# RC4ML/Legion

Measured on AMD Instinct MI355X. Metric: sampled_edges_per_sec, higher is better.
Workload: dtype int32+f32(copy)

## Files before the change

### legion_amd/csrc/kernels_sample.hip

```cpp
#include "legion_core.h"
#include "draw_rule.h"

#include <cstdlib>

namespace lg {

__global__ void draw_batch_kernel(const int32_t* idx, const int32_t* deg, int32_t* out, int32_t n)
{
    int32_t i = blockIdx.x * blockDim.x + threadIdx.x;
    if (i < n) out[i] = draw_from_x(minstd_pow((uint32_t)idx[i] + 1u), deg[i]);
}

void launch_draw_batch(hipStream_t s, const int32_t* idx, const int32_t* deg, int32_t* out, int32_t n)
{
    if (n <= 0) return;
    draw_batch_kernel<<<(n + 255) / 256, 256, 0, s>>>(idx, deg, out, n);
    hipCheckError();
}

__device__ __forceinline__ int32_t floyd_draw(uint32_t x, int32_t deg, int32_t f, int32_t k)
{
    return draw_from_x(x, deg - f + k + 1);
}

template <typename T>
__device__ __forceinline__ void floyd_resolve(T* p, int32_t n, int32_t jbase)
{
    for (int32_t k = 1; k < n; k++) {
        const int32_t t = p[k];
        bool taken = false;
        for (int32_t i = 0; i < k; i++) taken |= (p[i] == t);
        if (taken) p[k] = jbase + k;
    }
}

__global__ void draw_distinct_batch_kernel(const int32_t* base, const int32_t* deg, int32_t f, int32_t* out, int32_t n)
{
    const int32_t i = blockIdx.x * blockDim.x + threadIdx.x;
    if (i >= n) return;
    const int32_t D = deg[i] > 0 ? deg[i] : 0;
    int32_t* p = out + (int64_t)i * f;
    for (int32_t k = 0; k < f; k++)
        p[k] = k >= D ? -1 : (D <= f ? k : floyd_draw(minstd_pow((uint32_t)(base[i] + k) + 1u), D, f, k));
    if (D > f) floyd_resolve(p, f, D - f);
}

void launch_draw_distinct_batch(hipStream_t s, const int32_t* base, const int32_t* deg, int32_t f, int32_t* out, int32_t n)
{
    if (n <= 0) return;
    draw_distinct_batch_kernel<<<(n + 255) / 256, 256, 0, s>>>(base, deg, f, out, n);
    hipCheckError();
}

__global__ void draw_weighted_batch_kernel(const int32_t* idx, const int64_t* row_start, const int32_t* deg, const float* cdf, int32_t* out, int32_t n)
{
    const int32_t i = blockIdx.x * blockDim.x + threadIdx.x;
    if (i >= n) return;
    const int32_t D = deg[i];
    int32_t pick = -1;
    if (D > 0) {
        const float* c = cdf + row_start[i];
        const float T = c[D - 1];
        if (T > 0.0f) {
            const double t = weighted_target(minstd_pow((uint32_t)idx[i] + 1u), T);
            int32_t lo = 0, m = D;
            while (m > 0) weighted_step(c[lo + (m >> 1)], t, lo, m);
            pick = min(lo, D - 1);
        }
    }
    out[i] = pick;
}

void launch_draw_weighted_batch(hipStream_t s, const int32_t* idx, const int64_t* row_start, const int32_t* deg, const float* cdf, int32_t* out, int32_t n)
{
    if (n <= 0) return;
    draw_weighted_batch_kernel<<<(n + 255) / 256, 256, 0, s>>>(idx, row_start, deg, cdf, out, n);
    hipCheckError();
}

struct BracketLane {
    LG_G int32_t* sampled_ids; LG_G int32_t* labels; LG_G int32_t* node_counter; LG_G int32_t* edge_counter;
    LG_G int32_t* hop_scratch; LG_G int32_t* node_slot;
    LG_G int32_t* known_cnt; LG_G int32_t* claim_cnt; int32_t lds_buckets;
    LG_G int32_t* counter_mirror;
};
__device__ __forceinline__ BracketLane bracket_lane(const LanePtrs& P)
{
    BracketLane L;
    L.sampled_ids = LG_GPTR(int32_t, P.sampled_ids); L.labels = LG_GPTR(int32_t, P.labels);
    L.node_counter = LG_GPTR(int32_t, P.node_counter); L.edge_counter = LG_GPTR(int32_t, P.edge_counter);
    L.hop_scratch = LG_GPTR(int32_t, P.hop_scratch); L.node_slot = LG_GPTR(int32_t, P.node_slot);
    L.known_cnt = LG_GPTR(int32_t, P.known_cnt); L.claim_cnt = LG_GPTR(int32_t, P.claim_cnt); L.lds_buckets = P.lds_buckets;
    L.counter_mirror = LG_GPTR(int32_t, P.counter_mirror);
    return L;
}

__device__ __forceinline__ void raise_error(LG_G int32_t* hop_scratch, LG_G int32_t* err_flag, int32_t bits)
{
    __hip_atomic_fetch_or(hop_scratch + HS_ERROR, bits, __ATOMIC_RELAXED, __HIP_MEMORY_SCOPE_AGENT);
    if (err_flag) __hip_atomic_fetch_or(err_flag, bits, __ATOMIC_RELAXED, __HIP_MEMORY_SCOPE_SYSTEM);
}

__global__ void batch_generate_kernel(SeedParams p, const LanePtrs* __restrict__ lanes)
{
    const BracketLane L = bracket_lane(lanes[blockIdx.y]);
    const int32_t idx = blockIdx.x * blockDim.x + threadIdx.x;
    const int32_t counter = (p.iter_state != nullptr ? p.iter_state[0] : p.counter0) + (int32_t)blockIdx.y;
    const int32_t size = ((int64_t)p.batch_size * (counter + 1) >= p.total_cap)
                             ? (p.total_cap - p.batch_size * counter) : p.batch_size;
    if (L.known_cnt != nullptr && idx < L.lds_buckets) L.known_cnt[idx] = 0;
    if (L.claim_cnt != nullptr && idx < L.lds_buckets) L.claim_cnt[idx * LG_CLAIM_CNT_STRIDE] = 0;
    if (idx < 16) {
        int32_t v = 0;
        if (idx == 1) v = size;
        if (idx == INTRABATCH_CON * 3) v = size;
        if (idx == INTRABATCH_CON * 3 - 1) v = p.hop_num;
        L.node_counter[idx] = v;
        L.edge_counter[idx] = 0;
        if (idx == 0) {
            L.hop_scratch[HS_RANGE] = 0;
            L.hop_scratch[HS_RANGE + 1] = size;
        }
    }
    if (idx < size) {
        const int64_t at = (int64_t)size * counter + idx;
        if (at >= p.total_cap) {
            L.sampled_ids[idx] = -1;
            L.labels[idx] = -1;
        } else {
            const int32_t src_id = p.all_ids[at % p.total_cap];
            L.sampled_ids[idx] = src_id;
            if (L.node_slot != nullptr) L.node_slot[idx] = LG_FS_UNKNOWN;
            L.labels[idx] = p.all_labels[at % p.total_cap];
        }
    }
}

void launch_batch_generate(hipStream_t s, const SeedParams& p, const LanePtrs* d_lanes, int32_t n_lanes)
{
    const int32_t n = p.batch_size > 256 ? p.batch_size : 256;
    batch_generate_kernel<<<dim3((n + 255) / 256, n_lanes), 256, 0, s>>>(p, d_lanes);
    hipCheckError();
}

typedef int32_t lg_v4i __attribute__((ext_vector_type(4)));
typedef int32_t lg_v2i __attribute__((ext_vector_type(2)));
template <int NB> __device__ __forceinline__ int64_t lg_claim_at(int32_t b, int32_t k)
{
    return ((((int64_t)(k >> LG_CLAIM_CHUNK_BITS) * NB) + b) << LG_CLAIM_CHUNK_BITS) + (k & (LG_CLAIM_CHUNK - 1));
}
struct SampleArgs {
    int32_t op_id, count, partition_count, max_slots;
    int32_t* const* csr_dst_node_ids;
    int32_t* const* csr_dst_x;
    const LG_G int32_t* col_full; const LG_G lg_v2i* colx_full;
    const LG_G RowHdr* row_hdr;
    bool last_hop, is_presc;
    LG_G unsigned long long* edge_access_time;
    LG_G unsigned long long* topo_transactions;
    LG_G int32_t* sampled_ids; LG_G int32_t* agg_src_ids; LG_G int32_t* agg_dst_ids; LG_G int32_t* agg_src_off; LG_G int32_t* agg_dst_off;
    LG_G char* tmp_part_ind; LG_G int32_t* node_counter; LG_G int32_t* edge_counter;
    LG_G int32_t* slot_dst; LG_G int32_t* slot_pos; LG_G int32_t* slot_fs; LG_G int32_t* node_slot; LG_G unsigned long long* tile_state; LG_G int32_t* hop_scratch;
    LG_G RowHdr* fh_edge;
    LG_G int32_t* err_flag;
    LG_G unsigned long long* claim_pairs; LG_G int32_t* run_off; LG_G int32_t* claim_cnt; int32_t claim_cap, ids_cap;
    LG_G unsigned long long* known_pairs; LG_G int32_t* known_cnt; int32_t known_cap;
    const LG_G int64_t* indptr_full; LG_G int32_t* slot_pick; LG_G int64_t* agg_edge_ids;
    const LG_G float* edge_cdf;
};


__device__ __forceinline__ RowHdr load_hdr(const LG_G RowHdr* p)
{
    const lg_v4i t = *(const LG_G lg_v4i*)p;
    RowHdr h;
    h.start = (int64_t)(((uint64_t)(uint32_t)t.y << 32) | (uint32_t)t.x);
    h.deg = t.z;
    h.slot = t.w;
    return h;
}
__device__ __forceinline__ void store_hdr(LG_G RowHdr* p, const RowHdr& h)
{
    lg_v4i t;
    t.x = (int32_t)(uint32_t)h.start;
    t.y = (int32_t)((uint64_t)h.start >> 32);
    t.z = h.deg;
    t.w = h.slot;
    *(LG_G lg_v4i*)p = t;
}

__device__ __forceinline__ SampleArgs lane_args(const HopParams& p, const LanePtrs* __restrict__ lanes)
{
    const LanePtrs& L = lanes[blockIdx.y];
    SampleArgs a;
    a.op_id = p.op_id; a.count = p.count; a.partition_count = p.partition_count; a.max_slots = p.max_slots;
    a.csr_dst_node_ids = p.csr_dst_node_ids; a.csr_dst_x = p.csr_dst_x;
    a.col_full = LG_GPTR(const int32_t, p.col_full); a.colx_full = LG_GPTR(const lg_v2i, p.colx_full); a.row_hdr = LG_GPTR(const RowHdr, p.row_hdr); a.last_hop = p.last_hop; a.is_presc = p.is_presc;
    a.edge_access_time = LG_GPTR(unsigned long long, p.edge_access_time);
    a.topo_transactions = LG_GPTR(unsigned long long, p.topo_transactions);
    a.sampled_ids = LG_GPTR(int32_t, L.sampled_ids); a.agg_src_ids = LG_GPTR(int32_t, L.agg_src_ids);
    a.agg_dst_ids = LG_GPTR(int32_t, L.agg_dst_ids); a.agg_src_off = LG_GPTR(int32_t, L.agg_src_off);
    a.agg_dst_off = LG_GPTR(int32_t, L.agg_dst_off); a.tmp_part_ind = LG_GPTR(char, L.tmp_part_ind);
    a.node_counter = LG_GPTR(int32_t, L.node_counter);
    a.edge_counter = LG_GPTR(int32_t, L.edge_counter); a.slot_dst = LG_GPTR(int32_t, L.slot_dst);
    a.slot_pos = LG_GPTR(int32_t, L.slot_pos);
    a.slot_fs = LG_GPTR(int32_t, L.slot_fs); a.node_slot = LG_GPTR(int32_t, L.node_slot); a.tile_state = LG_GPTR(unsigned long long, L.tile_state); a.hop_scratch = LG_GPTR(int32_t, L.hop_scratch);
    a.fh_edge = LG_GPTR(RowHdr, L.fh_edge);
    a.err_flag = LG_GPTR(int32_t, L.err_flag);
    a.claim_pairs = LG_GPTR(unsigned long long, L.claim_pairs);
    a.run_off = LG_GPTR(int32_t, L.run_off);
    a.claim_cnt = LG_GPTR(int32_t, L.claim_cnt); a.claim_cap = L.claim_cap; a.ids_cap = L.ids_cap;
    a.known_pairs = LG_GPTR(unsigned long long, L.known_pairs); a.known_cnt = LG_GPTR(int32_t, L.known_cnt); a.known_cap = L.known_cap;
    a.indptr_full = LG_GPTR(const int64_t, p.indptr_full); a.slot_pick = LG_GPTR(int32_t, L.slot_pick);
    a.agg_edge_ids = LG_GPTR(int64_t, L.agg_edge_ids);
    a.edge_cdf = LG_GPTR(const float, p.edge_cdf);
    return a;
}

struct HopGeom {
    const LG_G int32_t* frontier;
    int32_t frontier_len;
    int32_t frontier_off;
    int32_t total;
    int32_t ntiles;
    int32_t nsuper;
};

__device__ __forceinline__ HopGeom hop_geometry(const SampleArgs& a)
{
    HopGeom g;
    if (a.op_id == INTRABATCH_CON) {
        g.frontier = a.sampled_ids;
        g.frontier_len = a.node_counter[1];
        g.frontier_off = 0;
    } else {
        g.frontier_off = a.edge_counter[0];
        g.frontier = a.agg_src_ids + g.frontier_off;
        g.frontier_len = a.edge_counter[1];
    }
    int64_t total = (int64_t)(g.frontier_len > 0 ? g.frontier_len : 0) * a.count;
    if (total > a.max_slots) total = a.max_slots;
    g.total = (int32_t)total;
    g.ntiles = (g.total + LG_TILE - 1) / LG_TILE;
    g.nsuper = (g.total + LG_SUPER - 1) / LG_SUPER;
    return g;
}

#ifndef LG_SAMPLE_SGPRS
#define LG_SAMPLE_SGPRS 80
#endif
template <int BB, bool SINGLE, bool STAGED, SampleDraw DRAW, bool EIDS>
__global__ __launch_bounds__(LG_TILE) __attribute__((amdgpu_num_sgpr(LG_SAMPLE_SGPRS))) void sample_kernel(HopParams hp, const LanePtrs* __restrict__ lanes)
{
    constexpr int NB = 1 << BB;
    constexpr bool DISTINCT = DRAW == SampleDraw::Distinct, WEIGHTED = DRAW == SampleDraw::Weighted;
    const int32_t K = SINGLE ? 1 : hp.lds_k;
    static_assert(NB <= LG_TILE, "one thread per bucket in the prefix");
    const SampleArgs a = lane_args(hp, lanes);
    __shared__ RowHdr s_hdr[LG_SUPER];
    __shared__ int32_t s_pick[DISTINCT ? LG_SUPER + LG_DISTINCT_MAX_FANOUT - 1 : 1];
    __shared__ int32_t s_bcnt[NB], s_boff[SINGLE ? NB : 1], s_list[STAGED ? NB : 1];
    static_assert(!STAGED || (SINGLE && NB <= 64), "the staged form scans its buckets with one wave");
    static_assert(!WEIGHTED || LG_SLOTS_PER_LANE == 4, "the lock-step search below names its four slots");

    const HopGeom g = hop_geometry(a);
    const int32_t tid = threadIdx.x;
    const int32_t count = a.count;
    const bool seeds = (a.op_id == INTRABATCH_CON);
    const LG_G RowHdr* fh = a.fh_edge + g.frontier_off;

    const int32_t nparts = (g.nsuper + K - 1) / K;
    for (int32_t m = blockIdx.x; m < nparts; m += gridDim.x) {
        if (!SINGLE && tid < NB) s_bcnt[tid] = 0;
        for (int32_t sub = 0; sub < K; sub++) {
            const int32_t st = m * K + sub;
            if (st >= g.nsuper) break;
            const int32_t idx0 = st * LG_SUPER;
            const int32_t last = min(idx0 + LG_SUPER - 1, g.total - 1);
            const int32_t j0 = idx0 / count;
            const int32_t nsrc = last / count - j0 + 1;

            uint32_t x[LG_SLOTS_PER_LANE];
#pragma unroll
            for (int u = 0; u < LG_SLOTS_PER_LANE; u++) x[u] = minstd_pow((uint32_t)(idx0 + u * LG_TILE + tid) + 1u);

            unsigned long long tx = 0;
            for (int32_t t = tid; t < nsrc; t += LG_TILE) {
                RowHdr h;
                bool real = true;
                if (seeds) {
                    const int32_t src = g.frontier[j0 + t];
                    if (src >= 0) {
                        h = load_hdr(a.row_hdr + src);
                    } else {
                        h.start = 0; h.deg = 0; h.slot = a.partition_count;
                        real = false;
                    }
                } else {
                    h = load_hdr(fh + j0 + t);
                }
                s_hdr[t] = h;
                if (a.topo_transactions && real && (int64_t)(j0 + t) * count >= idx0)
                    tx += 1ull + (unsigned long long)min(count, (h.deg * 4 + 63) / 64);
                if (!a.is_presc)
                    a.tmp_part_ind[j0 + t] = (char)(h.slot == a.partition_count ? CACHEMISS_FLAG : h.slot);
            }
            if (a.topo_transactions) {
                for (int off = 32; off > 0; off >>= 1) tx += __shfl_down(tx, off);
                if ((tid & 63) == 0 && tx != 0)
                    __hip_atomic_fetch_add(a.topo_transactions, tx, __ATOMIC_RELAXED, __HIP_MEMORY_SCOPE_AGENT);
            }
            __syncthreads();

            if constexpr (DISTINCT) {
                const int32_t sbase = j0 * count;
#pragma unroll
                for (int u = 0; u < LG_SLOTS_PER_LANE; u++) {
                    const int32_t idx = idx0 + u * LG_TILE + tid;
                    if (idx < g.total) {
                        const int32_t q = idx / count;
                        const int32_t k = idx - q * count;
                        const int32_t deg = s_hdr[q - j0].deg;
                        if (deg > count) s_pick[idx - sbase] = floyd_draw(x[u], deg, count, k);
                    }
                }
                __syncthreads();
                for (int32_t t = tid; t < nsrc; t += LG_TILE) {
                    const int32_t deg = s_hdr[t].deg;
                    if (deg <= count) continue;
                    if (t == 0)
                        for (int32_t k = 0; k < idx0 - sbase; k++) s_pick[k] = floyd_draw(minstd_pow((uint32_t)(sbase + k) + 1u), deg, count, k);
                    floyd_resolve(s_pick + t * count, min(count, last + 1 - (j0 + t) * count), deg - count);
                }
                __syncthreads();
            }

            if (SINGLE && tid < NB) s_bcnt[tid] = 0;
            int32_t dst[LG_SLOTS_PER_LANE], fs[LG_SLOTS_PER_LANE];
            int32_t pk[EIDS ? LG_SLOTS_PER_LANE : 1];
            int32_t wpick[WEIGHTED ? LG_SLOTS_PER_LANE : 1];
            if constexpr (WEIGHTED) {
                const LG_G float* wc[LG_SLOTS_PER_LANE];
                int32_t wn[LG_SLOTS_PER_LANE], wlo[LG_SLOTS_PER_LANE], wdeg[LG_SLOTS_PER_LANE];
                double wt[LG_SLOTS_PER_LANE];
#pragma unroll
                for (int u = 0; u < LG_SLOTS_PER_LANE; u++) {
                    const int32_t idx = idx0 + u * LG_TILE + tid;
                    wn[u] = 0; wlo[u] = 0; wdeg[u] = 0; wc[u] = a.edge_cdf;
                    if (idx < g.total) {
                        const int32_t q = idx / count;
                        const RowHdr h = s_hdr[q - j0];
                        if (idx - q * count < h.deg) {
                            const int64_t base = h.slot == a.partition_count ? h.start : a.indptr_full[g.frontier[q]];
                            wc[u] = a.edge_cdf + base;
                            wdeg[u] = h.deg;
                        }
                    }
                }
                float wtot[LG_SLOTS_PER_LANE];
#pragma unroll
                for (int u = 0; u < LG_SLOTS_PER_LANE; u++) wtot[u] = wdeg[u] > 0 ? wc[u][wdeg[u] - 1] : 0.0f;
#pragma unroll
                for (int u = 0; u < LG_SLOTS_PER_LANE; u++) {
                    wt[u] = weighted_target(x[u], wtot[u]);
                    if (wtot[u] > 0.0f) wn[u] = wdeg[u];
                }
                while ((wn[0] | wn[1] | wn[2] | wn[3]) != 0) {
                    float v[LG_SLOTS_PER_LANE];
#pragma unroll
                    for (int u = 0; u < LG_SLOTS_PER_LANE; u++) v[u] = wn[u] > 0 ? wc[u][wlo[u] + (wn[u] >> 1)] : 0.0f;
#pragma unroll
                    for (int u = 0; u < LG_SLOTS_PER_LANE; u++)
                        if (wn[u] > 0) weighted_step(v[u], wt[u], wlo[u], wn[u]);
                }
#pragma unroll
                for (int u = 0; u < LG_SLOTS_PER_LANE; u++) wpick[u] = wtot[u] > 0.0f ? min(wlo[u], wdeg[u] - 1) : -1;
            }
#pragma unroll
            for (int u = 0; u < LG_SLOTS_PER_LANE; u++) {
                const int32_t idx = idx0 + u * LG_TILE + tid;
                dst[u] = -1;
                fs[u] = LG_FS_UNKNOWN;
                if constexpr (EIDS) pk[u] = 0;
                if (idx < g.total) {
                    const int32_t q = idx / count;
                    const int32_t k = idx - q * count;
                    const RowHdr h = s_hdr[q - j0];
                    if (WEIGHTED ? wpick[u] >= 0 : k < h.deg) {
                        const int32_t pick = WEIGHTED ? wpick[u]
                                           : !DISTINCT ? draw_from_x(x[u], h.deg)
                                                       : (h.deg <= count ? k : s_pick[idx - j0 * count]);
                        const int64_t at = h.start + (int64_t)pick;
                        if constexpr (EIDS) pk[u] = pick;
                        if (h.slot == a.partition_count) {
                            if (a.colx_full != nullptr) {
                                const lg_v2i e = __builtin_nontemporal_load(&a.colx_full[at]);
                                dst[u] = e.x;
                                fs[u] = e.y;
                            } else {
                                dst[u] = __builtin_nontemporal_load(&a.col_full[at]);
                            }
                        } else {
                            const LG_G lg_v2i* cx = a.csr_dst_x != nullptr ? LG_GPTR(const lg_v2i, a.csr_dst_x[h.slot]) : nullptr;
                            if (cx != nullptr) {
                                const lg_v2i e = cx[at];
                                dst[u] = e.x;
                                fs[u] = e.y;
                            } else {
                                dst[u] = LG_GPTR(const int32_t, a.csr_dst_node_ids[h.slot])[at];
                            }
                        }
                    }
                }
            }
#pragma unroll
            for (int u = 0; u < LG_SLOTS_PER_LANE; u++) {
                const int32_t idx = idx0 + u * LG_TILE + tid;
                if (idx < g.total) {
                    if (dst[u] >= 0 && a.edge_access_time)
                        __hip_atomic_fetch_add(a.edge_access_time + g.frontier[idx / count], 1ull, __ATOMIC_RELAXED,
                                               __HIP_MEMORY_SCOPE_AGENT);
                    if (dst[u] < 0) dst[u] = -1;
                    __builtin_nontemporal_store(dst[u], &a.slot_dst[idx]);
                    a.slot_pos[idx] = -1;
                    if (a.slot_fs != nullptr && dst[u] >= 0) __builtin_nontemporal_store(fs[u], &a.slot_fs[idx]);
                    if constexpr (EIDS)
                        if (dst[u] >= 0) __builtin_nontemporal_store(pk[u], &a.slot_pick[idx]);
                }
            }
            if (SINGLE) {
                int32_t rank[LG_SLOTS_PER_LANE], bkt[LG_SLOTS_PER_LANE];
                __syncthreads();
#pragma unroll
                for (int u = 0; u < LG_SLOTS_PER_LANE; u++) {
                    bkt[u] = -1;
                    if (dst[u] >= 0) {
                        bkt[u] = (int32_t)(lg_tab_hash(dst[u]) & (NB - 1));
                        rank[u] = atomicAdd(&s_bcnt[bkt[u]], 1);
                    }
                }
                __syncthreads();
                if (STAGED) {
                    unsigned long long* s_stage = reinterpret_cast<unsigned long long*>(s_hdr);
                    if (tid < 64) {
                        const int32_t c = tid < NB ? s_bcnt[tid] : 0;
                        int32_t inc = c;
                        for (int d = 1; d < 64; d <<= 1) { const int32_t o = __shfl_up(inc, d); if (tid >= d) inc += o; }
                        if (tid < NB) {
                            s_boff[tid] = inc - c;
                            s_list[tid] = c > 0 ? __hip_atomic_fetch_add(a.claim_cnt + tid * LG_CLAIM_CNT_STRIDE, c, __ATOMIC_RELAXED, __HIP_MEMORY_SCOPE_AGENT) : 0;
                        }
                    }
                    __syncthreads();
#pragma unroll
                    for (int u = 0; u < LG_SLOTS_PER_LANE; u++)
                        if (bkt[u] >= 0)
                            s_stage[s_boff[bkt[u]] + rank[u]] = ((unsigned long long)(uint32_t)dst[u] << 32) | (uint32_t)(idx0 + u * LG_TILE + tid);
                    __syncthreads();
                    const int32_t tot = s_boff[NB - 1] + s_bcnt[NB - 1];
                    for (int32_t i = tid; i < tot; i += LG_TILE) {
                        const unsigned long long pr = s_stage[i];
                        const int32_t bk = (int32_t)(lg_tab_hash((int32_t)(pr >> 32)) & (NB - 1));
                        const int32_t at = s_list[bk] + (i - s_boff[bk]);
                        if (at < a.claim_cap) a.claim_pairs[lg_claim_at<NB>(bk, at)] = pr;
                    }
                } else {
                    if (tid < NB) {
                        const int32_t c = s_bcnt[tid];
                        s_boff[tid] = c > 0 ? __hip_atomic_fetch_add(a.claim_cnt + tid * LG_CLAIM_CNT_STRIDE, c, __ATOMIC_RELAXED, __HIP_MEMORY_SCOPE_AGENT) : 0;
                    }
                    __syncthreads();
#pragma unroll
                    for (int u = 0; u < LG_SLOTS_PER_LANE; u++)
                        if (bkt[u] >= 0) {
                            const int32_t at = s_boff[bkt[u]] + rank[u];
                            if (at < a.claim_cap)
                                a.claim_pairs[lg_claim_at<NB>(bkt[u], at)] =
                                    ((unsigned long long)(uint32_t)dst[u] << 32) | (uint32_t)(idx0 + u * LG_TILE + tid);
                        }
                }
            }

            if (!SINGLE) {
#pragma unroll
                for (int u = 0; u < LG_SLOTS_PER_LANE; u++)
                    if (dst[u] >= 0) atomicAdd(&s_bcnt[lg_tab_hash(dst[u]) & (NB - 1)], 1);
            }
            __syncthreads();
        }
        if (!SINGLE) {
            if (tid < NB) {
                const int32_t c = s_bcnt[tid];
                lg_v2i r;
                r.x = c > 0 ? __hip_atomic_fetch_add(a.claim_cnt + tid * LG_CLAIM_CNT_STRIDE, c, __ATOMIC_RELAXED, __HIP_MEMORY_SCOPE_AGENT) : 0;
                r.y = c;
                ((LG_G lg_v2i*)a.run_off)[(int64_t)m * NB + tid] = r;
            }
            __syncthreads();
        }
    }
}

#define LG_PLACE_THREADS 1024
template <int BB>
__global__ __launch_bounds__(LG_PLACE_THREADS) void place_kernel(HopParams hp, const LanePtrs* __restrict__ lanes)
{
    constexpr int NB = 1 << BB;
    static_assert(NB <= 256 && LG_SUPER == LG_PLACE_THREADS, "one thread per bucket in the prefix, one slot per thread and super tile");
    extern __shared__ unsigned long long s_stage[];
    __shared__ int32_t s_off[NB + 1], s_cnt[NB], s_list[NB], s_wtot[4];
    const SampleArgs a = lane_args(hp, lanes);
    const int32_t K = hp.lds_k;
    const HopGeom g = hop_geometry(a);
    const int32_t tid = threadIdx.x;
    const int32_t nparts = (g.nsuper + K - 1) / K;
    for (int32_t m = blockIdx.x; m < nparts; m += gridDim.x) {
        lg_v2i r; r.x = 0; r.y = 0;
        if (tid < NB) r = ((const LG_G lg_v2i*)a.run_off)[(int64_t)m * NB + tid];
        int32_t inc = r.y;
        if (tid < 256) {
            for (int d = 1; d < 64; d <<= 1) { const int32_t o = __shfl_up(inc, d); if ((tid & 63) >= d) inc += o; }
            if ((tid & 63) == 63) s_wtot[tid >> 6] = inc;
        }
        __syncthreads();
        int32_t wbase = 0, tot = 0;
        for (int w = 0; w < 4; w++) { if (w < (tid >> 6)) wbase += s_wtot[w]; tot += s_wtot[w]; }
        if (tid < NB) { s_off[tid] = wbase + inc - r.y; s_list[tid] = r.x; s_cnt[tid] = 0; }
        if (tid == 0) s_off[NB] = tot;
        __syncthreads();
        for (int32_t sub0 = 0; sub0 < K; sub0 += 4) {
            int32_t d[4];
#pragma unroll
            for (int u = 0; u < 4; u++) {
                const int32_t idx = (m * K + sub0 + u) * LG_SUPER + tid;
                d[u] = (sub0 + u < K && idx < g.total) ? a.slot_dst[idx] : -1;
            }
#pragma unroll
            for (int u = 0; u < 4; u++) {
                if (d[u] < 0) continue;
                const int32_t bk = (int32_t)(lg_tab_hash(d[u]) & (NB - 1));
                const int32_t rk = atomicAdd(&s_cnt[bk], 1);
                s_stage[s_off[bk] + rk] = ((unsigned long long)(uint32_t)d[u] << 32) | (uint32_t)((m * K + sub0 + u) * LG_SUPER + tid);
            }
        }
        __syncthreads();
        for (int32_t i = tid; i < tot; i += LG_PLACE_THREADS) {
            const unsigned long long pr = s_stage[i];
            const int32_t bk = (int32_t)(lg_tab_hash((int32_t)(pr >> 32)) & (NB - 1));
            const int32_t at = s_list[bk] + (i - s_off[bk]);
            if (at < a.claim_cap) a.claim_pairs[lg_claim_at<NB>(bk, at)] = pr;
        }
        __syncthreads();
    }
}

#ifndef LG_DEDUP_THREADS
#define LG_DEDUP_THREADS 1024
#endif

__device__ __forceinline__ void lds_barrier()
{
    __builtin_amdgcn_fence(__ATOMIC_RELEASE, "workgroup", "local");
    __builtin_amdgcn_s_barrier();
    __builtin_amdgcn_fence(__ATOMIC_ACQUIRE, "workgroup", "local");
}

template <int BB, int CL, int TB = LG_LDS_TABLE_BITS>
__global__ __launch_bounds__(LG_DEDUP_THREADS, (CL <= LG_DEDUP_CLAIMS_MID ? 8 : 4)) __attribute__((amdgpu_num_sgpr(80)))
void dedup_lists_kernel(HopParams hp, const LanePtrs* __restrict__ lanes)
{
    constexpr int NB = 1 << BB;
    constexpr uint32_t PENDING = 0x80000000u;
    constexpr int TABLE = 1 << TB;
    auto slot_of = [](uint32_t h) { return (h * 0x9E3779B1u) >> (32 - TB); };
    __shared__ unsigned long long s_tab[TABLE];
    __shared__ int32_t s_full;
    const int32_t tid = threadIdx.x, b = (int32_t)blockIdx.x;
    const SampleArgs a = lane_args(hp, lanes);

    unsigned long long rp[CL];
#pragma unroll
    for (int u = 0; u < CL; u++) {
        const int32_t k = u * LG_DEDUP_THREADS + tid;
        rp[u] = k < a.claim_cap ? a.claim_pairs[lg_claim_at<NB>(b, k)] : ~0ull;
    }
    unsigned long long kl0 = (a.known_pairs != nullptr && tid < a.known_cap) ? a.known_pairs[(int64_t)b * a.known_cap + tid] : ~0ull;
    const int32_t n_listed = a.known_pairs != nullptr ? a.known_cnt[b] : 0;
    const int32_t total = a.claim_cnt[b * LG_CLAIM_CNT_STRIDE];
    const int32_t kid0 = tid < a.ids_cap ? a.sampled_ids[tid] : -1;
    const int32_t n_known = a.node_counter[0] + a.node_counter[1];
    const int32_t n_seed = min(max(a.node_counter[INTRABATCH_CON * 3], 0), n_known);

    auto insert = [&](unsigned long long w, uint32_t h) {
        uint32_t p = slot_of(h);
        for (int it = 0; it < TABLE; it++) {
            const unsigned long long old = __hip_atomic_fetch_min(&s_tab[p], w, __ATOMIC_RELAXED, __HIP_MEMORY_SCOPE_WORKGROUP);
            if (old == ~0ull || (uint32_t)(old >> 32) == (uint32_t)(w >> 32)) return;
            if (old > w) w = old;
            p = (p + 1) & (TABLE - 1);
        }
        s_full = 1;
    };

    const bool listed = a.known_pairs != nullptr && n_listed <= a.known_cap;
    const int32_t n_scan = listed ? n_seed : n_known;
    const LG_G unsigned long long* klist = a.known_pairs + (int64_t)b * a.known_cap;
#pragma unroll
    for (int u = 0; u < CL; u++)
        if (u * LG_DEDUP_THREADS + tid >= total) rp[u] = ~0ull;
    if (!listed || tid >= n_listed) kl0 = ~0ull;
    const int32_t known_est = (listed ? n_listed : 0) + n_scan / NB + n_scan / (4 * NB) + 32;
    int32_t passes = 1;
    while ((int64_t)known_est + total > (int64_t)passes * (TABLE / 16 * LG_LDS_FILL_16THS)) passes <<= 1;
    const bool from_slots = total > a.claim_cap;
    const bool resident = !from_slots && total <= CL * LG_DEDUP_THREADS;
    const int32_t n_src = from_slots ? hop_geometry(a).total : total;
    auto fetch = [&](int32_t k0, unsigned long long (&pr)[CL]) {
#pragma unroll
        for (int u = 0; u < CL; u++) {
            const int32_t k = k0 + u * LG_DEDUP_THREADS + tid;
            pr[u] = ~0ull;
            if (k >= n_src) continue;
            if (from_slots) {
                int32_t d = a.slot_dst[k];
                if (d == -1) continue;
                if (d < -1) d = LG_SLOT_LOSER(d);
                if ((lg_tab_hash(d) & (NB - 1)) == (uint32_t)b) pr[u] = ((unsigned long long)(uint32_t)d << 32) | (uint32_t)k;
            } else {
                pr[u] = a.claim_pairs[lg_claim_at<NB>(b, k)];
            }
        }
    };

    for (;;) {
        const uint32_t pmask = (uint32_t)passes - 1u;
        bool overflow = false;
        for (uint32_t pass = 0; pass <= pmask; pass++) {
            for (int32_t i = tid; i < TABLE; i += LG_DEDUP_THREADS) s_tab[i] = ~0ull;
            if (tid == 0) s_full = 0;
            lds_barrier();
            for (int32_t i0 = 0; i0 < n_scan; i0 += LG_DEDUP_THREADS) {
                const int32_t i = i0 + tid;
                const int32_t id = i >= n_scan ? -1 : (i0 == 0 ? kid0 : a.sampled_ids[i]);
                if (id < 0) continue;
                const uint32_t h = lg_tab_hash(id);
                if ((h & (NB - 1)) != (uint32_t)b || ((h >> BB) & pmask) != pass) continue;
                insert(((unsigned long long)(uint32_t)id << 32) | (uint32_t)i, h);
            }
            if (listed)
                for (int32_t i0 = 0; i0 < n_listed; i0 += LG_DEDUP_THREADS) {
                    const int32_t i = i0 + tid;
                    const unsigned long long pr = i0 == 0 ? kl0 : (i < n_listed ? klist[i] : ~0ull);
                    if (pr == ~0ull) continue;
                    const uint32_t h = lg_tab_hash((int32_t)(pr >> 32));
                    if (((h >> BB) & pmask) != pass) continue;
                    insert(pr, h);
                }
            for (int32_t k0 = 0; k0 < n_src; k0 += CL * LG_DEDUP_THREADS) {
                unsigned long long pr[CL];
                if (resident) {
#pragma unroll
                    for (int u = 0; u < CL; u++) pr[u] = rp[u];
                } else
                    fetch(k0, pr);
#pragma unroll
                for (int u = 0; u < CL; u++) {
                    if (pr[u] == ~0ull) continue;
                    const uint32_t h = lg_tab_hash((int32_t)(pr[u] >> 32));
                    if (((h >> BB) & pmask) != pass) continue;
                    insert((pr[u] & 0xFFFFFFFF00000000ull) | PENDING | (uint32_t)pr[u], h);
                }
            }
            lds_barrier();
            if (s_full != 0) { overflow = true; break; }
            for (int32_t k0 = 0; k0 < n_src; k0 += CL * LG_DEDUP_THREADS) {
                unsigned long long pr[CL];
                if (resident) {
#pragma unroll
                    for (int u = 0; u < CL; u++) pr[u] = rp[u];
                } else
                    fetch(k0, pr);
#pragma unroll
                for (int u = 0; u < CL; u++) {
                    if (pr[u] == ~0ull) continue;
                    const uint32_t id = (uint32_t)(pr[u] >> 32), slot = (uint32_t)pr[u];
                    const uint32_t h = lg_tab_hash((int32_t)id);
                    if (((h >> BB) & pmask) != pass) continue;
                    uint32_t p = slot_of(h);
                    uint32_t v = 0xFFFFFFFFu;
                    for (int it = 0; it < TABLE; it++) {
                        const unsigned long long w = s_tab[p];
                        if ((uint32_t)(w >> 32) == id) { v = (uint32_t)w; break; }
                        p = (p + 1) & (TABLE - 1);
                    }
                    if (v != (PENDING | slot)) {
                        a.slot_dst[slot] = LG_SLOT_LOSER((int32_t)id);
                        a.slot_pos[slot] = (v & PENDING) ? -2 - (int32_t)(v & ~PENDING) : (int32_t)v;
                    }
                }
            }
            lds_barrier();
        }
        if (!overflow) break;
        if (passes >= (1 << 14)) {
            if (tid == 0) raise_error(a.hop_scratch, a.err_flag, LG_ERR_TABLE_FULL);
            break;
        }
        passes <<= 1;
        lds_barrier();
    }
    if (tid == 0) a.claim_cnt[b * LG_CLAIM_CNT_STRIDE] = 0;
}

#ifndef LG_SCATTER_MIN_WAVES
#define LG_SCATTER_MIN_WAVES 5
#endif
#ifndef LG_SCATTER_MIN_WAVES_LAST
#define LG_SCATTER_MIN_WAVES_LAST 8
#endif
#ifndef LG_SCATTER_MIN_WAVES_LAST_EIDS
#define LG_SCATTER_MIN_WAVES_LAST_EIDS 6
#endif
#define LG_SPIN_LIMIT (1 << 24)
#define LG_ST_AGG (1ull << 62)
#define LG_ST_PREF (2ull << 62)
__device__ __forceinline__ unsigned long long st_word(unsigned long long status, int32_t e, int32_t n)
{
    return status | ((unsigned long long)(uint32_t)e << 31) | (unsigned long long)(uint32_t)n;
}
__device__ __forceinline__ int32_t st_edges(unsigned long long w) { return (int32_t)((w >> 31) & 0x7FFFFFFFull); }
__device__ __forceinline__ int32_t st_nodes(unsigned long long w) { return (int32_t)(w & 0x7FFFFFFFull); }

template <bool LAST, int CT, bool EIDS = false>
__global__ __launch_bounds__(CT, LAST ? (EIDS ? LG_SCATTER_MIN_WAVES_LAST_EIDS : LG_SCATTER_MIN_WAVES_LAST) : LG_SCATTER_MIN_WAVES) __attribute__((amdgpu_num_sgpr(80)))
void compact_kernel(HopParams hp, const LanePtrs* __restrict__ lanes)
{
    constexpr int NW = LG_SLOTS_PER_LANE * (CT / 64);
    constexpr int CSUPER = LG_SLOTS_PER_LANE * CT;
    static_assert(NW <= 64, "one lane of wave 0 per (u, wave)");
    const SampleArgs a = lane_args(hp, lanes);
    __shared__ int32_t s_cnt[2][NW];
    __shared__ int32_t s_pre[2][NW];
    __shared__ unsigned long long s_mf[NW];
    __shared__ int32_t s_st, s_ex[2], s_last, s_tot[2];
    const HopGeom g = hop_geometry(a);
    LG_G int32_t* hs = a.hop_scratch;
    LG_G int32_t* nc = a.node_counter;
    LG_G int32_t* ec = a.edge_counter;
    const int32_t nc0 = nc[0], nc1 = nc[1], ec0 = ec[0], ec1 = ec[1];
    const int32_t total = g.total, nsuper = (g.total + CSUPER - 1) / CSUPER;
    const bool seeds = a.op_id == INTRABATCH_CON;
    const int32_t f_off = g.frontier_off;
    const int32_t node_base = nc0 + nc1, edge_base = ec0 + ec1;
    const LG_G int32_t* frontier = g.frontier;
    LG_G unsigned long long* state = a.tile_state;
    const int32_t tid = threadIdx.x;
    const int32_t wave = tid >> 6, lane = tid & 63;
    const unsigned long long lt = (lane == 0) ? 0ull : (~0ull >> (64 - lane));

    if (tid == 0) s_st = __hip_atomic_fetch_add(hs + HS_CTICKET, 1, __ATOMIC_RELAXED, __HIP_MEMORY_SCOPE_AGENT);
    __syncthreads();
    for (;;) {
        const int32_t st = s_st;
        if (st >= nsuper) break;
        const int32_t idx0 = st * CSUPER;
        int32_t v[LG_SLOTS_PER_LANE];
        unsigned long long mv[LG_SLOTS_PER_LANE], mf[LG_SLOTS_PER_LANE];
#pragma unroll
        for (int u = 0; u < LG_SLOTS_PER_LANE; u++) {
            const int32_t idx = idx0 + u * CT + tid;
            v[u] = idx < total ? a.slot_dst[idx] : -1;
        }
        int32_t src_of[LG_SLOTS_PER_LANE], src_pos[LG_SLOTS_PER_LANE], fsv[LG_SLOTS_PER_LANE];
        int32_t pk[EIDS ? LG_SLOTS_PER_LANE : 1];
        int64_t row0[EIDS ? LG_SLOTS_PER_LANE : 1];
#pragma unroll
        for (int u = 0; u < LG_SLOTS_PER_LANE; u++) {
            const int32_t idx = idx0 + u * CT + tid;
            src_of[u] = 0; src_pos[u] = 0; fsv[u] = LG_FS_UNKNOWN;
            if constexpr (EIDS) { pk[u] = 0; row0[u] = 0; }
            if (idx < total) {
                const int32_t q = idx / a.count;
                src_of[u] = frontier[q];
                src_pos[u] = seeds ? q : a.agg_src_off[f_off + q];
                if (a.slot_fs != nullptr) fsv[u] = a.slot_fs[idx];
                if constexpr (EIDS) pk[u] = a.slot_pick[idx];
            }
        }
        if constexpr (EIDS) {
#pragma unroll
            for (int u = 0; u < LG_SLOTS_PER_LANE; u++)
                if (idx0 + u * CT + tid < total && src_of[u] >= 0) row0[u] = a.indptr_full[src_of[u]];
        }
#pragma unroll
        for (int u = 0; u < LG_SLOTS_PER_LANE; u++) {
            const bool valid = v[u] != -1;
            const bool first = v[u] >= 0;
            if (v[u] < -1) v[u] = LG_SLOT_LOSER(v[u]);
            mv[u] = __ballot(valid);
            mf[u] = __ballot(first);
            if (lane == 0) {
                s_cnt[0][u * (CT / 64) + wave] = __popcll(mv[u]);
                s_cnt[1][u * (CT / 64) + wave] = __popcll(mf[u]);
                s_mf[u * (CT / 64) + wave] = mf[u];
            }
        }
        lds_barrier();
        int32_t te = 0, tn = 0;
        if (wave == 0) {
            const int32_t ce = lane < NW ? s_cnt[0][lane] : 0, cn = lane < NW ? s_cnt[1][lane] : 0;
            int32_t ie = ce, in = cn;
            for (int d = 1; d < NW; d <<= 1) {
                const int32_t oe = __shfl_up(ie, d), on = __shfl_up(in, d);
                if (lane >= d) { ie += oe; in += on; }
            }
            te = __shfl(ie, NW - 1);
            tn = __shfl(in, NW - 1);
            if (lane < NW) {
                s_pre[0][lane] = ie - ce;
                s_pre[1][lane] = in - cn;
            }
            if (st > 0 && lane == 0)
                __hip_atomic_store(state + st, st_word(LG_ST_AGG, te, tn), __ATOMIC_RELAXED, __HIP_MEMORY_SCOPE_AGENT);
        }
        int32_t lost_pos[LG_SLOTS_PER_LANE];
        RowHdr nh[LG_SLOTS_PER_LANE];
#pragma unroll
        for (int u = 0; u < LG_SLOTS_PER_LANE; u++) {
            const int32_t idx = idx0 + u * CT + tid;
            if constexpr (EIDS) row0[u] += (int64_t)pk[u];
            if (v[u] >= 0) {
                const bool first = (mf[u] >> lane) & 1ull;
                if (!first) fsv[u] = LG_FS_UNKNOWN;
                if (!LAST) nh[u] = load_hdr(a.row_hdr + v[u]);
                lost_pos[u] = first ? 0 : a.slot_pos[idx];
            }
        }
        if (wave == 0) {
            int32_t xe = 0, xn = 0;
            if (st > 0) {
                int32_t j = st - 1;
                for (;;) {
                    const int32_t me = j - lane;
                    unsigned long long w = LG_ST_PREF;
                    if (me >= 0) {
                        w = __hip_atomic_load(state + me, __ATOMIC_RELAXED, __HIP_MEMORY_SCOPE_AGENT);
                        for (int32_t spin = 0; (w >> 62) == 0; spin++) {
                            if (spin == LG_SPIN_LIMIT) {
                                raise_error(a.hop_scratch, a.err_flag, LG_ERR_CHAIN);
                                w = LG_ST_AGG;
                                break;
                            }
                            __builtin_amdgcn_s_sleep(1);
                            w = __hip_atomic_load(state + me, __ATOMIC_RELAXED, __HIP_MEMORY_SCOPE_AGENT);
                        }
                    }
                    const unsigned long long pm = __ballot((w >> 62) == 2);
                    const int first_p = pm ? __builtin_ctzll(pm) : 64;
                    if (lane <= first_p) { xe += st_edges(w); xn += st_nodes(w); }
                    if (pm) break;
                    j -= 64;
                }
                for (int off = 32; off > 0; off >>= 1) { xe += __shfl_down(xe, off); xn += __shfl_down(xn, off); }
                xe = __shfl(xe, 0);
                xn = __shfl(xn, 0);
            }
            if (lane == 0) {
                s_ex[0] = xe;
                s_ex[1] = xn;
                __hip_atomic_store(state + st, st_word(LG_ST_PREF, xe + te, xn + tn), __ATOMIC_RELAXED, __HIP_MEMORY_SCOPE_AGENT);
            }
        }
        lds_barrier();
        const int32_t xe = s_ex[0], xn = s_ex[1];
        int32_t n_at[LG_SLOTS_PER_LANE];
#pragma unroll
        for (int u = 0; u < LG_SLOTS_PER_LANE; u++) {
            n_at[u] = -1;
            if ((mf[u] >> lane) & 1ull) {
                n_at[u] = node_base + xn + s_pre[1][u * (CT / 64) + wave] + __popcll(mf[u] & lt);
                __hip_atomic_store(a.slot_pos + idx0 + u * CT + tid, n_at[u], __ATOMIC_RELAXED, __HIP_MEMORY_SCOPE_AGENT);
            }
        }
        {
#pragma unroll
            for (int u = 0; u < LG_SLOTS_PER_LANE; u++) {
                if (v[u] < 0 || lost_pos[u] >= -1) continue;
                const int32_t w = -2 - lost_pos[u];
                if (w >= idx0) {
                    const int32_t ww = (w - idx0) >> 6, lw = w & 63;
                    lost_pos[u] = node_base + xn + s_pre[1][ww] + __popcll(s_mf[ww] & (lw == 0 ? 0ull : (~0ull >> (64 - lw))));
                } else {
                    const LG_G int32_t* wp = a.slot_pos + w;
                    int32_t np = __hip_atomic_load(wp, __ATOMIC_RELAXED, __HIP_MEMORY_SCOPE_AGENT);
                    for (int32_t spin = 0; np < 0; spin++) {
                        if (spin == LG_SPIN_LIMIT) {
                            raise_error(a.hop_scratch, a.err_flag, LG_ERR_CHAIN);
                            np = 0;
                            break;
                        }
                        __builtin_amdgcn_s_sleep(1);
                        np = __hip_atomic_load(wp, __ATOMIC_RELAXED, __HIP_MEMORY_SCOPE_AGENT);
                    }
                    lost_pos[u] = np;
                }
            }
        }
        int32_t next_st = 0;
        if (tid == 0) next_st = __hip_atomic_fetch_add(hs + HS_CTICKET, 1, __ATOMIC_RELAXED, __HIP_MEMORY_SCOPE_AGENT);
#pragma unroll
        for (int u = 0; u < LG_SLOTS_PER_LANE; u++) {
            if (v[u] < 0) continue;
            const int32_t dst = v[u];
            const int32_t e = edge_base + xe + s_pre[0][u * (CT / 64) + wave] + __popcll(mv[u] & lt);
#ifdef LG_COMPACT_NO_NT
            constexpr bool NT = false;
#else
            constexpr bool NT = LAST;
#endif
            if (NT) {
                __builtin_nontemporal_store(dst, &a.agg_src_ids[e]);
                __builtin_nontemporal_store(src_of[u], &a.agg_dst_ids[e]);
                __builtin_nontemporal_store(src_pos[u], &a.agg_dst_off[e]);
            } else {
                a.agg_src_ids[e] = dst;
                a.agg_dst_ids[e] = src_of[u];
                a.agg_dst_off[e] = src_pos[u];
            }
            if constexpr (EIDS) {
                if (NT) __builtin_nontemporal_store(row0[u], &a.agg_edge_ids[e]);
                else a.agg_edge_ids[e] = row0[u];
            }
            if (!LAST) store_hdr(a.fh_edge + e, nh[u]);
            const int32_t n = n_at[u];
            if (n >= 0) {
                a.sampled_ids[n] = dst;
                if (a.node_slot != nullptr) a.node_slot[n] = fsv[u];
                if (NT) __builtin_nontemporal_store(n, &a.agg_src_off[e]);
                else a.agg_src_off[e] = n;
            } else {
                if (NT) __builtin_nontemporal_store(lost_pos[u], &a.agg_src_off[e]);
                else a.agg_src_off[e] = lost_pos[u];
            }
        }
        if (tid == 0) s_st = next_st;
        lds_barrier();
    }

    if (tid == 0) {
        __builtin_amdgcn_s_waitcnt(0x0F70);
        s_last = (__hip_atomic_fetch_add(hs + HS_CDONE, 1, __ATOMIC_RELAXED, __HIP_MEMORY_SCOPE_AGENT) == (int32_t)gridDim.x - 1) ? 1 : 0;
    }
    __syncthreads();
    if (!s_last) return;
    if (tid == 0) {
        const unsigned long long tw = nsuper > 0 ? __hip_atomic_load(state + nsuper - 1, __ATOMIC_RELAXED, __HIP_MEMORY_SCOPE_AGENT) : 0ull;
        s_tot[0] = st_edges(tw);
        s_tot[1] = st_nodes(tw);
    }
    __syncthreads();
    for (int32_t t = tid; t < nsuper; t += CT) state[t] = 0ull;
    if (tid == 0) {
        const int32_t n_edge = s_tot[0], n_new = s_tot[1];
        hs[HS_CTICKET] = 0;
        hs[HS_CDONE] = 0;
        hs[HS_FRONTIER_IS_SEEDS] = seeds ? 1 : 0;
        hs[HS_FRONTIER_OFF] = f_off;
        hs[HS_FRONTIER_LEN] = g.frontier_len;
        hs[HS_NODE_BASE] = node_base;
        hs[HS_EDGE_BASE] = edge_base;
        hs[HS_N_NEW] = n_new;
        hs[HS_N_EDGE] = n_edge;
        hs[HS_SLOTS] = total;
        const int32_t h = a.op_id / INTRABATCH_CON;
        hs[HS_RANGE + 2 * h] = node_base;
        hs[HS_RANGE + 2 * h + 1] = n_new;
        nc[0] = node_base;
        nc[1] = n_new;
        nc[INTRABATCH_CON * 2] = 0;
        nc[INTRABATCH_CON * 2 + 1] = node_base + n_new;
        ec[0] = edge_base;
        ec[1] = n_edge;
        ec[2] = 0;
        nc[INTRABATCH_CON * 3 + h] = node_base + n_new;
        ec[INTRABATCH_CON * 3 + h] = edge_base + n_edge;
    }
}

template <int BB>
__global__ __launch_bounds__(LG_TILE) void list_known_kernel(HopParams hp, const LanePtrs* __restrict__ lanes)
{
    constexpr int NB = 1 << BB;
    const SampleArgs a = lane_args(hp, lanes);
    __shared__ int32_t s_kcnt[NB], s_kbase[NB];
    if (a.known_pairs == nullptr) return;
    const int32_t tid = threadIdx.x;
    const int32_t h = a.op_id / INTRABATCH_CON;
    const int32_t base = a.hop_scratch[HS_RANGE + 2 * h], n_new = a.hop_scratch[HS_RANGE + 2 * h + 1];
    for (int32_t c0 = blockIdx.x * LG_LIST_CHUNK; c0 < n_new; c0 += gridDim.x * LG_LIST_CHUNK) {
        const int32_t c1 = min(c0 + LG_LIST_CHUNK, n_new);
        for (int32_t i = tid; i < NB; i += LG_TILE) s_kcnt[i] = 0;
        __syncthreads();
        for (int32_t i = c0 + tid; i < c1; i += LG_TILE)
            atomicAdd(&s_kcnt[lg_tab_hash(a.sampled_ids[base + i]) & (NB - 1)], 1);
        __syncthreads();
        for (int32_t i = tid; i < NB; i += LG_TILE) {
            const int32_t c = s_kcnt[i];
            s_kbase[i] = c ? __hip_atomic_fetch_add(a.known_cnt + i, c, __ATOMIC_RELAXED, __HIP_MEMORY_SCOPE_AGENT) : 0;
            s_kcnt[i] = 0;
        }
        __syncthreads();
        for (int32_t i = c0 + tid; i < c1; i += LG_TILE) {
            const int32_t id = a.sampled_ids[base + i];
            const int32_t bk = (int32_t)(lg_tab_hash(id) & (NB - 1));
            const int32_t at = s_kbase[bk] + atomicAdd(&s_kcnt[bk], 1);
            if (at < a.known_cap)
                a.known_pairs[(int64_t)bk * a.known_cap + at] = ((unsigned long long)(uint32_t)id << 32) | (uint32_t)(base + i);
        }
        __syncthreads();
    }
}

template <int BB, int CL>
static bool launch_dedup(hipStream_t s, const SampleHopPlan& plan, const HopParams& q, const LanePtrs* d_lanes, int32_t n_lanes)
{
    if constexpr (CL <= sample_class(BB).max_claims) {
        if (plan.dedup_claims == CL) {
            dedup_lists_kernel<BB, CL, lg_dedup_table_bits(CL)><<<dim3(1 << BB, n_lanes), LG_DEDUP_THREADS, 0, s>>>(q, d_lanes);
            return true;
        }
    }
    return false;
}

template <int BB, SampleDraw DRAW>
static void launch_sample(hipStream_t s, dim3 grid, const HopParams& q, const LanePtrs* d_lanes)
{
    constexpr SampleClassInfo ci = sample_class(BB);
    if (q.mode.edge_ids) sample_kernel<BB, ci.single, ci.staged, DRAW, true><<<grid, LG_TILE, 0, s>>>(q, d_lanes);
    else sample_kernel<BB, ci.single, ci.staged, DRAW, false><<<grid, LG_TILE, 0, s>>>(q, d_lanes);
}
template <bool EIDS>
static void launch_compact(hipStream_t s, dim3 grid, const HopParams& p, const LanePtrs* d_lanes)
{
    if (p.last_hop) compact_kernel<true, LG_COMPACT_THREADS, EIDS><<<grid, LG_COMPACT_THREADS, 0, s>>>(p, d_lanes);
    else compact_kernel<false, LG_COMPACT_THREADS, EIDS><<<grid, LG_COMPACT_THREADS, 0, s>>>(p, d_lanes);
}

template <int BB>
static void launch_hop(hipStream_t s, const SampleHopPlan& plan, const HopParams& p, const LanePtrs* d_lanes, int32_t n_lanes)
{
    constexpr SampleClassInfo ci = sample_class(BB);
    HopParams q = p;
    q.lds_k = plan.k;
    const dim3 grid(plan.sample_gx, n_lanes);
    switch (p.mode.draw()) {
    case SampleDraw::Uniform: launch_sample<BB, SampleDraw::Uniform>(s, grid, q, d_lanes); break;
    case SampleDraw::Distinct: launch_sample<BB, SampleDraw::Distinct>(s, grid, q, d_lanes); break;
    case SampleDraw::Weighted: launch_sample<BB, SampleDraw::Weighted>(s, grid, q, d_lanes); break;
    }
    hipCheckError();
    if constexpr (!ci.single) {
        place_kernel<BB><<<dim3(plan.place_gx, n_lanes), LG_PLACE_THREADS, (size_t)plan.stage_bytes, s>>>(q, d_lanes);
        hipCheckError();
    }
    if (!launch_dedup<BB, LG_DEDUP_CLAIMS_BIG>(s, plan, q, d_lanes, n_lanes) && !launch_dedup<BB, LG_DEDUP_CLAIMS_MID>(s, plan, q, d_lanes, n_lanes) &&
        !launch_dedup<BB, LG_DEDUP_CLAIMS>(s, plan, q, d_lanes, n_lanes)) {
        printf("legion_hip: no dedup_lists_kernel for %d buckets and %d claims per thread\n", 1 << BB, plan.dedup_claims);
        exit(EXIT_FAILURE);
    }
    hipCheckError();
    const dim3 cgrid(plan.compact_gx, n_lanes);
    if (p.mode.edge_ids) launch_compact<true>(s, cgrid, p, d_lanes);
    else launch_compact<false>(s, cgrid, p, d_lanes);
    hipCheckError();
    if (!p.last_hop) {
        list_known_kernel<BB><<<dim3(plan.known_chunks, n_lanes), LG_TILE, 0, s>>>(p, d_lanes);
        hipCheckError();
    }
}

void launch_random_sample(hipStream_t s, const HopParams& p, int32_t bucket_bits, int64_t last_hop_claims_hint, const LanePtrs* d_lanes,
                          int32_t n_lanes)
{
    const LegionTuning tune = tuning();
    const SampleHopPlan plan = sample_hop_plan(bucket_bits, p.max_slots, n_lanes, p.last_hop, last_hop_claims_hint, tune.sample_max_wg, tune.lds_part_wg);
    switch (sample_class(bucket_bits).bits) {
    case LG_LDS_BITS_SMALL: return launch_hop<LG_LDS_BITS_SMALL>(s, plan, p, d_lanes, n_lanes);
    case LG_LDS_BITS_SMALL16: return launch_hop<LG_LDS_BITS_SMALL16>(s, plan, p, d_lanes, n_lanes);
    case LG_LDS_BITS_MEDIUM: return launch_hop<LG_LDS_BITS_MEDIUM>(s, plan, p, d_lanes, n_lanes);
    default: return launch_hop<LG_LDS_BITS_LARGE>(s, plan, p, d_lanes, n_lanes);
    }
}

__global__ void init_row_hdr_kernel(RowHdr* __restrict__ hdr, const int64_t* __restrict__ csr_index, int32_t n,
                                    int32_t slot)
{
    for (int32_t v = blockIdx.x * blockDim.x + threadIdx.x; v < n; v += gridDim.x * blockDim.x) {
        RowHdr h;
        h.start = csr_index[v];
        h.deg = (int32_t)(csr_index[v + 1] - h.start);
        h.slot = slot;
        hdr[v] = h;
    }
}

void init_row_headers(hipStream_t s, RowHdr* hdr, const int64_t* csr_index, int32_t n, int32_t slot)
{
    int32_t grid = (n + 255) / 256;
    if (grid > 4096) grid = 4096;
    if (grid < 1) grid = 1;
    init_row_hdr_kernel<<<grid, 256, 0, s>>>(hdr, csr_index, n, slot);
    hipCheckError();
}

__global__ void cache_row_hdr_kernel(RowHdr* __restrict__ hdr, const int32_t* __restrict__ QT, int32_t Kg, int32_t Ki,
                                     int32_t capacity, int32_t n, const int64_t* __restrict__ d_index, int32_t slot)
{
    for (int32_t r = blockIdx.x * blockDim.x + threadIdx.x; r < capacity; r += gridDim.x * blockDim.x) {
        const int64_t t = (int64_t)r * Kg + Ki;
        if (t >= n) continue;
        RowHdr h;
        h.start = d_index[r];
        h.deg = (int32_t)(d_index[r + 1] - h.start);
        h.slot = slot;
        hdr[QT[t]] = h;
    }
}

void cache_row_headers(hipStream_t s, RowHdr* hdr, const int32_t* QT, int32_t Kg, int32_t Ki, int32_t capacity,
                       int32_t n, const int64_t* d_index, int32_t slot)
{
    if (capacity <= 0) return;
    int32_t grid = (capacity + 255) / 256;
    if (grid > 4096) grid = 4096;
    cache_row_hdr_kernel<<<grid, 256, 0, s>>>(hdr, QT, Kg, Ki, capacity, n, d_index, slot);
    hipCheckError();
}

__global__ void end_of_batch_kernel(const LanePtrs* __restrict__ lanes, int32_t* __restrict__ iter_state)
{
    const BracketLane L = bracket_lane(lanes[blockIdx.y]);
    if (L.counter_mirror != nullptr && threadIdx.x < 32) {
        const int32_t t = threadIdx.x;
        int32_t v = t < 16 ? L.node_counter[t] : L.edge_counter[t - 16];
        const int32_t hop_num = L.node_counter[INTRABATCH_CON * 3 - 1];
        if (t == 2 && hop_num >= 0 && hop_num <= 6) v = L.hop_scratch[HS_RANGE + 2 * hop_num];
        if (t == 3 && hop_num >= 0 && hop_num <= 6) v = L.hop_scratch[HS_RANGE + 2 * hop_num + 1];
        L.counter_mirror[t] = v;
    }
    if (iter_state != nullptr && blockIdx.y == 0 && threadIdx.x == 0) iter_state[0] += iter_state[1];
}

void launch_end_of_batch(hipStream_t s, const LanePtrs* d_lanes, int32_t n_lanes, int32_t* iter_state)
{
    end_of_batch_kernel<<<dim3(1, n_lanes), 64, 0, s>>>(d_lanes, iter_state);
    hipCheckError();
}

__global__ void hotness_measure_kernel(const int32_t* __restrict__ ids, const int32_t* __restrict__ nc,
                                       unsigned long long* __restrict__ access_map)
{
    const int32_t n = nc[INTRABATCH_CON * 2 + 1];
    for (int32_t i = blockIdx.x * blockDim.x + threadIdx.x; i < n; i += gridDim.x * blockDim.x) {
        const int32_t cid = ids[i];
        if (cid >= 0) atomicAdd(access_map + cid, 1ull);
    }
}

void launch_hotness_measure(hipStream_t s, const int32_t* sampled_ids, const int32_t* node_counter,
                            unsigned long long* access_map)
{
    hotness_measure_kernel<<<1024, 256, 0, s>>>(sampled_ids, node_counter, access_map);
    hipCheckError();
}

__global__ void find_kernel(const int32_t* __restrict__ keys, int32_t n,
                            const int32_t* __restrict__ map32, const char* __restrict__ map8,
                            int32_t* __restrict__ out32, char* __restrict__ out8)
{
    for (int32_t i = blockIdx.x * blockDim.x + threadIdx.x; i < n; i += gridDim.x * blockDim.x) {
        const int32_t k = keys[i];
        if (out32) out32[i] = (k >= 0 && map32) ? map32[k] : CACHEMISS_FLAG;
        if (out8) out8[i] = (k >= 0 && map8) ? map8[k] : (char)CACHEMISS_FLAG;
    }
}

void launch_find(hipStream_t s, const int32_t* keys, int32_t n, const int32_t* map32, const char* map8,
                 int32_t* out32, char* out8)
{
    if (n <= 0) return;
    int32_t grid = (n + 255) / 256;
    if (grid > 2048) grid = 2048;
    find_kernel<<<grid, 256, 0, s>>>(keys, n, map32, map8, out32, out8);
    hipCheckError();
}

}
```

Baseline: 5.580 billion.

## Publish last-hop slot positions as packed per-32-slot records instead of per-slot writes

```diff
diff --git a/legion_amd/csrc/kernels_sample.hip b/legion_amd/csrc/kernels_sample.hip
--- a/legion_amd/csrc/kernels_sample.hip
+++ b/legion_amd/csrc/kernels_sample.hip
@@ -422,7 +422,7 @@
                                                __HIP_MEMORY_SCOPE_AGENT);
                     if (dst[u] < 0) dst[u] = -1;
                     __builtin_nontemporal_store(dst[u], &a.slot_dst[idx]);
-                    a.slot_pos[idx] = -1;
+                    if (!a.last_hop) a.slot_pos[idx] = -1;
                     if (a.slot_fs != nullptr && dst[u] >= 0) __builtin_nontemporal_store(fs[u], &a.slot_fs[idx]);
                     if constexpr (EIDS)
                         if (dst[u] >= 0) __builtin_nontemporal_store(pk[u], &a.slot_pick[idx]);
@@ -565,6 +565,22 @@
     __builtin_amdgcn_fence(__ATOMIC_ACQUIRE, "workgroup", "local");
 }
 
+#define LG_REC_VALID (1ull << 63)
+static_assert(sizeof(RowHdr) >= sizeof(unsigned long long),
+              "a slot's entry of fh_edge holds more than its share of a record, and one seed's entry the record a partial group rounds up to");
+__device__ __forceinline__ LG_G unsigned long long* hop_records(const SampleArgs& a, int32_t edge_base)
+{
+    return (LG_G unsigned long long*)(a.fh_edge + edge_base);
+}
+__device__ __forceinline__ unsigned long long rec_word(int32_t prefix, uint32_t bits)
+{
+    return LG_REC_VALID | ((unsigned long long)(uint32_t)prefix << 32) | bits;
+}
+__device__ __forceinline__ int32_t rec_position(unsigned long long r, int32_t w)
+{
+    return (int32_t)((r >> 32) & 0x7FFFFFFFull) + __popc((uint32_t)r & ((1u << (w & 31)) - 1u));
+}
+
 template <int BB, int CL, int TB = LG_LDS_TABLE_BITS>
 __global__ __launch_bounds__(LG_DEDUP_THREADS, (CL <= LG_DEDUP_CLAIMS_MID ? 8 : 4)) __attribute__((amdgpu_num_sgpr(80)))
 void dedup_lists_kernel(HopParams hp, const LanePtrs* __restrict__ lanes)
@@ -590,6 +606,11 @@
     const int32_t kid0 = tid < a.ids_cap ? a.sampled_ids[tid] : -1;
     const int32_t n_known = a.node_counter[0] + a.node_counter[1];
     const int32_t n_seed = min(max(a.node_counter[INTRABATCH_CON * 3], 0), n_known);
+    if (a.last_hop) {
+        const int32_t words = (hop_geometry(a).total + 31) >> 5;
+        LG_G unsigned long long* rec = hop_records(a, a.edge_counter[0] + a.edge_counter[1]);
+        for (int32_t i = b * LG_DEDUP_THREADS + tid; i < words; i += NB * LG_DEDUP_THREADS) rec[i] = 0ull;
+    }
 
     auto insert = [&](unsigned long long w, uint32_t h) {
         uint32_t p = slot_of(h);
@@ -754,6 +775,7 @@
     const int32_t node_base = nc0 + nc1, edge_base = ec0 + ec1;
     const LG_G int32_t* frontier = g.frontier;
     LG_G unsigned long long* state = a.tile_state;
+    LG_G unsigned long long* records = hop_records(a, edge_base);
     const int32_t tid = threadIdx.x;
     const int32_t wave = tid >> 6, lane = tid & 63;
     const unsigned long long lt = (lane == 0) ? 0ull : (~0ull >> (64 - lane));
@@ -876,10 +898,18 @@
         int32_t n_at[LG_SLOTS_PER_LANE];
 #pragma unroll
         for (int u = 0; u < LG_SLOTS_PER_LANE; u++) {
+            const int32_t row_at = node_base + xn + s_pre[1][u * (CT / 64) + wave];
             n_at[u] = -1;
             if ((mf[u] >> lane) & 1ull) {
-                n_at[u] = node_base + xn + s_pre[1][u * (CT / 64) + wave] + __popcll(mf[u] & lt);
-                __hip_atomic_store(a.slot_pos + idx0 + u * CT + tid, n_at[u], __ATOMIC_RELAXED, __HIP_MEMORY_SCOPE_AGENT);
+                n_at[u] = row_at + __popcll(mf[u] & lt);
+                if constexpr (!LAST)
+                    __hip_atomic_store(a.slot_pos + idx0 + u * CT + tid, n_at[u], __ATOMIC_RELAXED, __HIP_MEMORY_SCOPE_AGENT);
+            }
+            if constexpr (LAST) {
+                const int32_t s0 = idx0 + u * CT + tid;
+                if ((lane & 31) == 0 && s0 < total)
+                    __hip_atomic_store(records + (s0 >> 5), rec_word(row_at + __popcll(mf[u] & lt), (uint32_t)(mf[u] >> lane)), __ATOMIC_RELAXED,
+                                       __HIP_MEMORY_SCOPE_AGENT);
             }
         }
         {
@@ -890,6 +920,19 @@
                 if (w >= idx0) {
                     const int32_t ww = (w - idx0) >> 6, lw = w & 63;
                     lost_pos[u] = node_base + xn + s_pre[1][ww] + __popcll(s_mf[ww] & (lw == 0 ? 0ull : (~0ull >> (64 - lw))));
+                } else if constexpr (LAST) {
+                    const LG_G unsigned long long* rp = records + (w >> 5);
+                    unsigned long long r = __hip_atomic_load(rp, __ATOMIC_RELAXED, __HIP_MEMORY_SCOPE_AGENT);
+                    for (int32_t spin = 0; (r & LG_REC_VALID) == 0; spin++) {
+                        if (spin == LG_SPIN_LIMIT) {
+                            raise_error(a.hop_scratch, a.err_flag, LG_ERR_CHAIN);
+                            r = LG_REC_VALID;
+                            break;
+                        }
+                        __builtin_amdgcn_s_sleep(1);
+                        r = __hip_atomic_load(rp, __ATOMIC_RELAXED, __HIP_MEMORY_SCOPE_AGENT);
+                    }
+                    lost_pos[u] = rec_position(r, w);
                 } else {
                     const LG_G int32_t* wp = a.slot_pos + w;
                     int32_t np = __hip_atomic_load(wp, __ATOMIC_RELAXED, __HIP_MEMORY_SCOPE_AGENT);
```

Result: slower. 5.521 billion (-1.1%).
